# isl-org/adaptive-surface-reconstruction

Measured on AMD Instinct MI355X. Metric: input points/sec to signed implicit values, higher is better.
Workload: dtype f32 via bf16x3 (24-bit operands, f32 accumulate)

## Files before the change

adaptive-surface-reconstruction_amd/csrc/asr_common.h:

```cpp
#pragma once
#include <hip/hip_runtime.h>

#include <cstdint>
#include <cstdio>
#include <map>
#include <string>
#include <tuple>
#include <vector>

#include "../../include/asr_hip.h"
#include "asr_pending.h"

typedef uint64_t u64;
typedef int64_t i64;
typedef uint32_t u32;

struct Arena {
    struct Slab {
        char* base;
        size_t size, used;
    };
    std::vector<Slab> slabs;
    size_t min_slab = size_t(256) << 20;
    size_t cap = 0;
    uint64_t generation = 0;

    void* alloc(size_t bytes) {
        bytes = (bytes + 255) & ~size_t(255);
        if (bytes == 0) bytes = 256;
        for (auto& s : slabs)
            if (s.size - s.used >= bytes) {
                void* p = s.base + s.used;
                s.used += bytes;
                return p;
            }
        size_t sz = bytes > min_slab ? bytes : min_slab;
        if (cap && reserved() + sz > cap) return nullptr;
        void* p = nullptr;
        if (hipMalloc(&p, sz) != hipSuccess) return nullptr;
        slabs.push_back({(char*)p, sz, bytes});
        return p;
    }
    void reset() {
        for (auto& s : slabs) s.used = 0;
        ++generation;
    }
    size_t reserved() const {
        size_t t = 0;
        for (auto& s : slabs) t += s.size;
        return t;
    }
    void release() {
        for (auto& s : slabs) (void)hipFree(s.base);
        slabs.clear();
    }
};

struct ArenaMark {
    std::vector<size_t> used;
};
static inline void arena_mark(const Arena& a, ArenaMark& m) {
    m.used.clear();
    for (auto& s : a.slabs) m.used.push_back(s.used);
}
static inline void arena_rewind(Arena& a, const ArenaMark& m) {
    for (size_t i = 0; i < a.slabs.size(); ++i) a.slabs[i].used = i < m.used.size() ? m.used[i] : 0;
    ++a.generation;
}

struct GridDev {
    i64 v = 0, p = 0;
    u64* keys = nullptr;
    float* centers = nullptr;
    float* sizes = nullptr;
    int32_t* nidx = nullptr;
    uint8_t* nkidx = nullptr;
    i64* nrs = nullptr;
    int32_t* up_idx = nullptr;
    uint8_t* up_kidx = nullptr;
    i64* up_rs = nullptr;
    int32_t* down_idx = nullptr;
    uint8_t* down_kidx = nullptr;
    i64* down_rs = nullptr;
    int32_t* perm_nb = nullptr;
    int32_t* perm_up = nullptr;
    int32_t* perm_down = nullptr;
};

struct AsrOptions {
    i64 sconv_min_blocks = 2816;
    i64 sconv16_min_blocks = 1024;
    i64 sconv_wide_min = 2048;
    i64 row_segment = 524288;
    i64 search_hash_level = -1;
    i64 knn_deep = 1;
    i64 knn_cells = 1;
    i64 plan_arena = 0;
    i64 sconv_plan = 1;
    i64 row_ranked = 1;
    i64 row_lpt = 1;
    i64 overlap = 1;
    i64 cconv_valu = 0;
    i64 build_search = 1;
    i64 shard_geometry = -1;
    i64 shard_timing = 0;
    i64 search_priority = 2;
    i64 search_half = 1;
    i64 early_cells = 1;
    i64 early_sort = 1;
    i64 arena_cap_mb = 0;
    i64 inject_failure = 0;
    i64 sconv_split_min_rows = 2048;
    i64 sconv_split_rows = 32768;
};

struct asr_conv_plan_view {
    const uint4* hdr;
    const int32_t* pool;
    i64 groups;
    unsigned pool_bytes;
};
struct asr_conv_plan {
    uint4* hdr = nullptr;
    int32_t* pool = nullptr;
// ... 403 lines not shown
```

adaptive-surface-reconstruction_amd/csrc/asr_geom.hip:

```cpp
#include <cstdlib>
#include <cstring>
#include <algorithm>
#include <rocprim/rocprim.hpp>

#include "asr_common.h"
#include "asr_prim.h"

namespace {
using namespace asr_prim;

constexpr int BLK = 256;

struct HashTab {
    u64* keys;
    int32_t* vals;
    u64 mask;
};

struct TabProbe {
    u64 bucket, step, low, bmask;
    __device__ inline u64 slot() const { return ((bucket & bmask) << 6) | low; }
    __device__ inline void next() { bucket += step; }
};
__device__ inline TabProbe tab_probe(const HashTab& t, u64 key) {
    const u64 h = asr_hash64(key >> 6);
    return TabProbe{h, (h >> 32) | 1, key & 63, t.mask >> 6};
}

__device__ inline u64 ld_agent(const u64* p) {
    return __hip_atomic_load(p, __ATOMIC_RELAXED, __HIP_MEMORY_SCOPE_AGENT);
}

__device__ inline int tab_insert(const HashTab& t, u64 key, u64* slot_out = nullptr) {
    TabProbe pr = tab_probe(t, key);
    for (u64 probe = 0; probe <= pr.bmask; ++probe, pr.next()) {
        const u64 slot = pr.slot();
        u64 cur = ld_agent(&t.keys[slot]);
        if (cur == 0) {
            cur = atomicCAS((unsigned long long*)&t.keys[slot], 0ull, (unsigned long long)key);
            if (cur == 0) {
                if (slot_out) *slot_out = slot;
                return 1;
            }
        }
        if (cur == key) {
            if (slot_out) *slot_out = slot;
            return 0;
        }
    }
    return -1;
}
__device__ inline int tab_insert_shared(const HashTab& t, u64 key) {
    TabProbe pr = tab_probe(t, key);
    for (u64 probe = 0; probe <= pr.bmask; ++probe, pr.next()) {
        const u64 slot = pr.slot();
        u64 cur = t.keys[slot];
        if (cur == 0) cur = ld_agent(&t.keys[slot]);
        if (cur == 0) {
            cur = atomicCAS((unsigned long long*)&t.keys[slot], 0ull, (unsigned long long)key);
            if (cur == 0) return 1;
        }
        if (cur == key) return 0;
    }
    return -1;
}
__device__ inline bool tab_contains(const HashTab& t, u64 key) {
    TabProbe pr = tab_probe(t, key);
    for (u64 probe = 0; probe <= pr.bmask; ++probe, pr.next()) {
        const u64 slot = pr.slot();
        const u64 cur = t.keys[slot];
        if (cur == key) return true;
        if (cur == 0) return false;
    }
    return false;
}
__device__ inline int tab_find(const HashTab& t, u64 key) {
    TabProbe pr = tab_probe(t, key);
    for (u64 probe = 0; probe <= pr.bmask; ++probe, pr.next()) {
        const u64 slot = pr.slot();
        const u64 cur = t.keys[slot];
        if (cur == key) return t.vals[slot];
        if (cur == 0) return -1;
    }
    return -1;
}
__device__ inline i64 tab_find_slot(const HashTab& t, u64 key) {
    TabProbe pr = tab_probe(t, key);
    for (u64 probe = 0; probe <= pr.bmask; ++probe, pr.next()) {
        const u64 slot = pr.slot();
        const u64 cur = t.keys[slot];
        if (cur == key) return (i64)slot;
        if (cur == 0) return -1;
    }
    return -1;
// ... 105 lines not shown
            key = point_key(f, pts, radii, i, radius_scale, max_depth);
    }
    const u64 left = __shfl_up(key, 1, 64);
    if ((threadIdx.x & 63) != 0 && left == key) return;
    if (key == 0) return;
    insert_with_ancestors(t, key, cnt, list, list_cap);
}

__global__ void k_grow_init(asr_octree_frame f, const float* pts, const float* radii, i64 n, float radius_scale,
                            int max_depth, HashTab t, int* cnt, u64* list, int list_cap) {
    i64 i = blockIdx.x * (i64)blockDim.x + threadIdx.x;
    if (i >= n) return;
    if (!(isfinite(pts[3 * i]) && isfinite(pts[3 * i + 1]) && isfinite(pts[3 * i + 2]) && isfinite(radii[i]))) {
        cnt[F_NONFINITE] = 1;
        return;
    }
    const u64 key = point_key(f, pts, radii, i, radius_scale, max_depth);
    if (key == 0) return;
    const int r = tab_insert(t, key);
    if (r < 0) cnt[F_OVERFLOW] = 1;
    if (r == 1) {
        const int pos = atomicAdd(&cnt[F_ENTRIES], 1);
        if (pos < list_cap)
            list[pos] = key;
        else
            cnt[F_OVERFLOW] = 1;
    }
}
__device__ inline bool tab_has_child(const HashTab& t, u64 key) {
    if (__clzll((long long)key) <= 1) return false;
    for (int k = 0; k < 8; ++k)
        if (tab_contains(t, (key << 3) + k)) return true;
    return false;
}
__global__ void k_grow_candidates(HashTab t, const u64* list, int lo, int count, u64* cand) {
    const int e = blockIdx.x * blockDim.x + threadIdx.x;
    if (e >= count * 7) return;
    const u64 cur = list[lo + e / 7];
    u64 out = 0;
    if (cur != 1) {
        const int cfg = 7 - (int)(cur & 7);
        int j = e % 7;
        if (j >= cfg) ++j;
        int x, y, z, lev;
        asr_key_coord(cur >> 3, x, y, z, lev);
        const u64 key = asr_coord_key(x + (j & 1) - (cfg & 1), y + ((j >> 1) & 1) - ((cfg >> 1) & 1),
                                      z + ((j >> 2) & 1) - ((cfg >> 2) & 1), lev);
        if (key != 0 && !tab_contains(t, key) && !tab_has_child(t, key)) out = key;
    }
    cand[e] = out;
}
__global__ void k_grow_insert(HashTab t, u64* list, int lo, int count, const u64* cand, int* cnt, int list_cap) {
    const int e = blockIdx.x * blockDim.x + threadIdx.x;
    if (e >= count * 14) return;
    const u64 cur = list[lo + e / 14];
    if (cur == 1) return;
    const int j = e % 14;
    u64 key;
    if (j < 7) {
        key = cand[(e / 14) * 7 + j];
        if (key == 0) return;
    } else {
        const u64 first = cur & ~u64(7);
        int sj = j - 7;
        if (first + sj >= cur) ++sj;
        key = first + sj;
    }
    const int r = tab_insert(t, key);
    if (r < 0) cnt[F_OVERFLOW] = 1;
    if (r == 1) {
        const int pos = atomicAdd(&cnt[F_ENTRIES], 1);
        if (pos < list_cap)
            list[pos] = key;
        else
            cnt[F_OVERFLOW] = 1;
    }
}
__global__ void k_octree_insert_keys(const u64* keys, i64 n, HashTab t, int* cnt, u64* list, int list_cap) {
    i64 i = blockIdx.x * (i64)blockDim.x + threadIdx.x;
    if (i >= n) return;
    insert_with_ancestors(t, keys[i], cnt, list, list_cap);
}

__global__ void k_balance_classify(HashTab t, const u64* list, int lo, int ngroups, uint8_t* flag) {
    int i = blockIdx.x * blockDim.x + threadIdx.x;
    if (i >= ngroups) return;
    u64 k = list[lo + 8 * i];
    bool has_child = (__clzll((long long)k) > 1) && tab_contains(t, k << 3);
    flag[i] = has_child ? 0 : 1;
}
__global__ void k_balance_insert(HashTab t, u64* list, int lo, int ngroups, const uint8_t* flag,
                                 int* cnt, int list_cap) {
    int i = blockIdx.x * blockDim.x + threadIdx.x;
    if (i >= ngroups * 6) return;
    if (!flag[i / 6]) return;
    u64 k = list[lo + 8 * (i / 6)];
    int j = i % 6;
    const int ox = (j == 0) ? -1 : (j == 3) ? 1 : 0;
    const int oy = (j == 1) ? -1 : (j == 4) ? 1 : 0;
    const int oz = (j == 2) ? -1 : (j == 5) ? 1 : 0;
    int x, y, z, lev;
    asr_key_coord(k >> 3, x, y, z, lev);
    u64 key = asr_coord_key(x + ox, y + oy, z + oz, lev);
    if (key == 0) return;
    insert_with_ancestors(t, key, cnt, list, list_cap);
}
__global__ void k_leaf_flags(HashTab t, const u64* nodes, i64 n, uint8_t* flags) {
    i64 i = blockIdx.x * (i64)blockDim.x + threadIdx.x;
    if (i >= n) return;
    const u64 k = nodes[i];
    flags[i] = (k != 0 && !((__clzll((long long)k) > 1) && tab_contains(t, k << 3))) ? 1 : 0;
}

__global__ void k_leaf_tail(const u64* leaves, const i64* num, i64* out3) {
    const i64 n = *num;
    out3[0] = n;
    out3[1] = n > 0 ? (i64)leaves[0] : 0;
    out3[2] = n > 0 ? (i64)leaves[n - 1] : 0;
}

__global__ void k_map_build(const u64* keys, i64 v, HashTab t, int* cnt) {
    i64 i = blockIdx.x * (i64)blockDim.x + threadIdx.x;
    if (i >= v) return;
    u64 slot;
    int r = tab_insert(t, keys[i], &slot);
    if (r < 0)
        cnt[F_OVERFLOW] = 1;
    else
        t.vals[slot] = (int32_t)i;
}

__constant__ int8_t c_child_off[24][3] = {
        {-1, 0, 0}, {-1, 1, 0}, {-1, 0, 1}, {-1, 1, 1}, {2, 0, 0},  {2, 1, 0},  {2, 0, 1},  {2, 1, 1},
        {0, -1, 0}, {1, -1, 0}, {0, -1, 1}, {1, -1, 1}, {0, 2, 0},  {1, 2, 0},  {0, 2, 1},  {1, 2, 1},
        {0, 0, -1}, {1, 0, -1}, {0, 1, -1}, {1, 1, -1}, {0, 0, 2},  {1, 0, 2},  {0, 1, 2},  {1, 1, 2}};
__constant__ int8_t c_nb_off[6][3] = {{-1, 0, 0}, {1, 0, 0}, {0, -1, 0},
                                      {0, 1, 0},  {0, 0, -1}, {0, 0, 1}};
__constant__ int8_t c_parent_koff[6][8] = {
        {-1, 0, -1, 1, -1, 2, -1, 3}, {0, -1, 1, -1, 2, -1, 3, -1}, {-1, -1, 0, 1, -1, -1, 2, 3},
        {0, 1, -1, -1, 2, 3, -1, -1}, {-1, -1, -1, -1, 0, 1, 2, 3}, {0, 1, 2, 3, -1, -1, -1, -1}};

__device__ inline int neighbor_candidate(const HashTab& t, u64 key, int x, int y, int z, int lev,
                                         int c, int& slot) {
    if (c < 6) {
        u64 nk = asr_coord_key(x + c_nb_off[c][0], y + c_nb_off[c][1], z + c_nb_off[c][2], lev);
        slot = 1 + c;
        return nk ? tab_find(t, nk) : -1;
    } else if (c < 30) {
        if (lev >= ASR_MAX_LEVEL) return -1;
        int j = c - 6;
        u64 nk = asr_coord_key(2 * x + c_child_off[j][0], 2 * y + c_child_off[j][1],
                               2 * z + c_child_off[j][2], lev + 1);
        slot = 7 + j;
        return nk ? tab_find(t, nk) : -1;
    } else {
        if (lev <= 0) return -1;
        int j = c - 30;
        u64 nk = asr_coord_key(x + c_nb_off[j][0], y + c_nb_off[j][1], z + c_nb_off[j][2], lev);
        if (!nk) return -1;
        int koff = c_parent_koff[j][nk & 7];
        if (koff < 0) return -1;
        slot = 31 + 4 * j + koff;
        return tab_find(t, nk >> 3);
    }
}

__global__ void k_check_rows(const int32_t* rows, i64 nrows, i64 v, int* cnt, int32_t* mark) {
    const i64 r = blockIdx.x * (i64)blockDim.x + threadIdx.x;
    if (r >= nrows) return;
    const i64 q = rows[r];
    if (q < 0 || q >= v || (r > 0 && rows[r - 1] >= q)) cnt[F_BAD_KEY] = 1;
    else if (mark) mark[q] = 1;
}
__global__ void k_check_keys(const u64* keys, i64 n, int* cnt) {
    const i64 i = blockIdx.x * (i64)blockDim.x + threadIdx.x;
    if (i >= n) return;
    const u64 k = keys[i];
    if (k == 0 || (63 - __clzll((long long)k)) % 3 != 0) cnt[F_BAD_KEY] = 1;
}

constexpr int NB_STAGE = 16;
constexpr int NB_MAX_JOBS = 8;
struct NbBatch {
    int n;
    i64 base[NB_MAX_JOBS + 1];
    i64 v[NB_MAX_JOBS];
    const u64* keys[NB_MAX_JOBS];
    HashTab tab[NB_MAX_JOBS];
    i64* rs[NB_MAX_JOBS];
// ... 1896 lines not shown
    t.keys = arena_alloc<u64>(arena, cap);
    t.vals = with_vals ? arena_alloc<int32_t>(arena, cap) : nullptr;
    t.mask = cap - 1;
    if (!t.keys || (with_vals && !t.vals)) ASR_FAIL(ctx, ASR_HIP_EHIP, "arena allocation failed");
    ASR_HIP_CHECK(ctx, hipMemsetAsync(t.keys, 0, cap * sizeof(u64), ctx->stream));
    return ASR_HIP_OK;
}

}

int asr_geom_point_keys(asr_hip_context* ctx, const asr_octree_frame* frame, const float* pts,
                        const float* radii, i64 n, float radius_scale, int max_depth, u64* keys) {
    if (n <= 0) return ASR_HIP_OK;
    k_point_keys<<<grid_for(n, BLK), BLK, 0, ctx->stream>>>(*frame, pts, radii, n, radius_scale,
                                                            max_depth, keys);
    ASR_CHECK_LAUNCH(ctx);
    return ASR_HIP_OK;
}

static int grow_keys(asr_hip_context* ctx, Arena& arena, const asr_octree_frame* frame, const float* pts, const float* radii,
                     i64 n, float radius_scale, int max_depth, int grow_steps, u64** keys_out, i64* count_out) {
    HostFlags host;
    u64 cap = next_pow2((u64)std::max<i64>(i64(1) << 16, 8 * n));
    for (int attempt = 0; attempt < 6; ++attempt, cap <<= 2) {
        if (attempt) ++ctx->table_regrows;
        HashTab t;
        ASR_TRY(make_table(ctx, arena, cap, false, t));
        const int lcap = (int)std::min<u64>(cap / 2, u64(1) << 30);
        u64* list = arena_alloc<u64>(arena, (size_t)lcap + 8);
        if (!list) ASR_FAIL(ctx, ASR_HIP_EHIP, "arena allocation failed");
        ASR_TRY(fresh_flags(ctx));
        k_grow_init<<<grid_for(n, BLK), BLK, 0, ctx->stream>>>(*frame, pts, radii, n, radius_scale, max_depth, t,
                                                             ctx->d_flags, list, lcap);
        ASR_CHECK_LAUNCH(ctx);
        ASR_TRY(read_flags(ctx, host));
        if (host[F_BAD_KEY]) ASR_FAIL(ctx, ASR_HIP_EINVAL, "octree: extra_keys holds a value that is no location code (0 or a leading "
                                                   "bit that is not at 3 * level)");
        if (host[F_NONFINITE]) ASR_FAIL(ctx, ASR_HIP_EINVAL, "octree: points / radii contain non-finite values");
        bool overflow = host[F_OVERFLOW] != 0;
        int lo = 0, hi = host[F_ENTRIES];
        for (int it = 0; it < grow_steps && !overflow && hi > lo; ++it) {
            const int count = hi - lo;
            if ((i64)count * 14 >= (i64(1) << 31) || (u64)(hi + (i64)count * 14) > (u64)lcap) {
                overflow = true;
                break;
            }
            u64* cand = arena_alloc<u64>(arena, (size_t)count * 7);
            if (!cand) ASR_FAIL(ctx, ASR_HIP_EHIP, "arena allocation failed");
            k_grow_candidates<<<grid_for((i64)count * 7, BLK), BLK, 0, ctx->stream>>>(t, list, lo, count, cand);
            ASR_CHECK_LAUNCH(ctx);
            k_grow_insert<<<grid_for((i64)count * 14, BLK), BLK, 0, ctx->stream>>>(t, list, lo, count, cand, ctx->d_flags,
                                                                                  lcap);
            ASR_CHECK_LAUNCH(ctx);
            ASR_TRY(read_flags(ctx, host));
            overflow = host[F_OVERFLOW] != 0;
            lo = hi;
            hi = host[F_ENTRIES];
        }
        if (overflow) continue;
        *keys_out = list;
        *count_out = host[F_ENTRIES];
        return ASR_HIP_OK;
    }
    ASR_FAIL(ctx, ASR_HIP_ELOGIC, "octree grow: hash table overflow");
}

int asr_geom_octree_build(asr_hip_context* ctx, const asr_octree_frame* frame, const float* pts,
                          const float* radii, i64 n, float radius_scale, int max_depth, int grow_steps,
                          const u64* extra_keys, i64 num_extra, bool balance) {
    ASR_TRY(ensure_flags(ctx));
    if (max_depth > ASR_MAX_LEVEL) max_depth = ASR_MAX_LEVEL;
    if (max_depth < 0) ASR_FAIL(ctx, ASR_HIP_EINVAL, "max_depth must be >= 0");
    if (grow_steps < 0) ASR_FAIL(ctx, ASR_HIP_EINVAL, "grow_steps must be >= 0");
    u64* grown = nullptr;
    i64 num_grown = 0;
    Arena grow_arena;
    grow_arena.min_slab = size_t(16) << 20;
    struct ArenaGuard {
        Arena& a;
        ~ArenaGuard() { a.release(); }
    } grow_guard{grow_arena};
    if (grow_steps > 0 && n > 0)
        ASR_TRY(grow_keys(ctx, grow_arena, frame, pts, radii, n, radius_scale, max_depth, grow_steps, &grown, &num_grown));
    u64 cap = next_pow2((u64)std::max<i64>(i64(1) << 16, 2 * std::max(std::max(n, 4 * num_grown), num_extra)));
    HostFlags host;
    for (int attempt = 0; attempt < 7; ++attempt, cap <<= 2) {
        if (attempt) ++ctx->table_regrows;
        ctx->scratch.reset();
        HashTab t;
        ASR_TRY(make_table(ctx, ctx->scratch, cap, false, t));
        int lcap = (int)std::min<u64>(cap / 2, u64(1) << 30);
        u64* list = arena_alloc<u64>(ctx->scratch, (size_t)lcap + 8);
        uint8_t* flag = arena_alloc<uint8_t>(ctx->scratch, (size_t)lcap / 8 + 8);
        if (!list || !flag) ASR_FAIL(ctx, ASR_HIP_EHIP, "arena allocation failed");
        ASR_TRY(fresh_flags(ctx));
        if (grown) {
            if (num_grown > 0)
                k_octree_insert_keys<<<grid_for(num_grown, BLK), BLK, 0, ctx->stream>>>(grown, num_grown, t, ctx->d_flags,
                                                                                       list, lcap);
            ASR_CHECK_LAUNCH(ctx);
        } else if (n > 0) {
            k_octree_insert_points<<<grid_for(n, BLK), BLK, 0, ctx->stream>>>(*frame, pts, radii, n, radius_scale, max_depth,
                                                                              t, ctx->d_flags, list, lcap);
            ASR_CHECK_LAUNCH(ctx);
        }
        if (num_extra > 0) {
            k_check_keys<<<grid_for(num_extra, BLK), BLK, 0, ctx->stream>>>(extra_keys, num_extra, ctx->d_flags);
            ASR_CHECK_LAUNCH(ctx);
            k_octree_insert_keys<<<grid_for(num_extra, BLK), BLK, 0, ctx->stream>>>(extra_keys, num_extra, t, ctx->d_flags,
                                                                                   list, lcap);
            ASR_CHECK_LAUNCH(ctx);
        }
        k_list_key_bits<<<256, BLK, 0, ctx->stream>>>(list, lcap, ctx->d_flags);
        ASR_CHECK_LAUNCH(ctx);
        ASR_TRY(read_flags(ctx, host));
        if (host[F_NONFINITE]) ASR_FAIL(ctx, ASR_HIP_EINVAL, "octree: points / radii contain non-finite values");
        bool overflow = host[F_OVERFLOW] != 0 || (u64)host[F_ENTRIES] * 2 > cap;
        int lo = 0, hi = host[F_ENTRIES];
        while (balance && !overflow && hi > lo) {
            int ngroups = (hi - lo) / 8;
            k_balance_classify<<<grid_for(ngroups, BLK), BLK, 0, ctx->stream>>>(t, list, lo, ngroups, flag);
            ASR_CHECK_LAUNCH(ctx);
            k_balance_insert<<<grid_for((i64)ngroups * 6, BLK), BLK, 0, ctx->stream>>>(
                    t, list, lo, ngroups, flag, ctx->d_flags, lcap);
            ASR_CHECK_LAUNCH(ctx);
            ASR_TRY(read_flags(ctx, host));
            overflow = host[F_OVERFLOW] != 0 || (u64)host[F_ENTRIES] * 2 > cap;
            lo = hi;
            hi = host[F_ENTRIES];
        }
        if (overflow) continue;
        i64 num_nodes = (i64)host[F_ENTRIES] + (host[F_ROOT] ? 1 : 0);
        ctx->leaf_lmin = ctx->leaf_lmax = -1;
        if (num_nodes == 0) {
            ctx->num_nodes = ctx->num_leaves = 0;
            ctx->nodes = ctx->leaves = nullptr;
            return ASR_HIP_OK;
        }
        if (host[F_ROOT]) {
            const u64 one = 1;
            ASR_HIP_CHECK(ctx, hipMemcpyAsync(list + host[F_ENTRIES], &one, sizeof(u64), hipMemcpyHostToDevice,
                                              ctx->stream));
        }
        ctx->nodes = arena_alloc<u64>(ctx->persist, num_nodes);
        u64* leaves_tmp = arena_alloc<u64>(ctx->scratch, num_nodes);
        uint8_t* lflag = arena_alloc<uint8_t>(ctx->scratch, num_nodes);
        i64* d_num = arena_alloc<i64>(ctx->scratch, 1);
        if (!ctx->nodes || !leaves_tmp || !lflag || !d_num) ASR_FAIL(ctx, ASR_HIP_EHIP, "arena allocation failed");
        ASR_TRY(sort_keys(ctx, ctx->scratch, list, ctx->nodes, num_nodes, host[F_KEY_BITS] > 0 && host[F_KEY_BITS] <= 64 ? host[F_KEY_BITS] : 64));
        k_leaf_flags<<<grid_for(num_nodes, BLK), BLK, 0, ctx->stream>>>(t, ctx->nodes, num_nodes, lflag);
        ASR_CHECK_LAUNCH(ctx);
        {
            size_t tb = 0;
            ASR_HIP_CHECK(ctx, rocprim::select(nullptr, tb, ctx->nodes, lflag, leaves_tmp, d_num, (size_t)num_nodes,
                                               ctx->stream));
            void* tmp = ctx->scratch.alloc(tb ? tb : 256);
            if (!tmp) ASR_FAIL(ctx, ASR_HIP_EHIP, "arena allocation failed");
            ASR_HIP_CHECK(ctx, rocprim::select(tmp, tb, ctx->nodes, lflag, leaves_tmp, d_num, (size_t)num_nodes,
                                               ctx->stream));
        }
        i64* d_tail = arena_alloc<i64>(ctx->scratch, 3);
        if (!d_tail) ASR_FAIL(ctx, ASR_HIP_EHIP, "arena allocation failed");
        k_leaf_tail<<<1, 1, 0, ctx->stream>>>(leaves_tmp, d_num, d_tail);
        ASR_CHECK_LAUNCH(ctx);
        i64 tail[3] = {0, 0, 0};
        ASR_HIP_CHECK(ctx, hipMemcpyAsync(tail, d_tail, sizeof(tail), hipMemcpyDeviceToHost, ctx->stream));
        ASR_HIP_CHECK(ctx, hipStreamSynchronize(ctx->stream));
        const i64 num_leaves = tail[0];
        auto level_of = [](u64 k) { return k ? (63 - __builtin_clzll(k)) / 3 : 0; };
        ctx->leaf_lmin = level_of((u64)tail[1]);
        ctx->leaf_lmax = level_of((u64)tail[2]);
        ctx->leaves = arena_alloc<u64>(ctx->persist, num_leaves);
        if (!ctx->leaves) ASR_FAIL(ctx, ASR_HIP_EHIP, "arena allocation failed");
        ASR_HIP_CHECK(ctx, hipMemcpyAsync(ctx->leaves, leaves_tmp, 8 * num_leaves, hipMemcpyDeviceToDevice, ctx->stream));
        ctx->num_nodes = num_nodes;
        ctx->num_leaves = num_leaves;
        return ASR_HIP_OK;
    }
    ASR_FAIL(ctx, ASR_HIP_ELOGIC, "octree hash table overflow after 6 growth attempts");
}

template <class Pass>
static int nb_key_maps(asr_hip_context* ctx, NbBatch& b, Pass&& pass, int grow0 = 0, int* grow_out = nullptr) {
    ASR_TRY(ensure_flags(ctx));
    for (int grow = grow0;; grow += 2) {
        u64 caps[NB_MAX_JOBS], cap_sum = 0;
        for (int j = 0; j < b.n; ++j) {
            caps[j] = next_pow2((u64)std::max<i64>(1024, 2 * b.v[j])) << grow;
            cap_sum += caps[j];
        }
        u64* tkeys = arena_alloc<u64>(ctx->scratch, cap_sum);
        int32_t* tvals = arena_alloc<int32_t>(ctx->scratch, cap_sum);
        if (!tkeys || !tvals) ASR_FAIL(ctx, ASR_HIP_EHIP, "arena allocation failed");
        u64 off = 0;
        for (int j = 0; j < b.n; ++j) {
            b.tab[j] = HashTab{tkeys + off, tvals + off, caps[j] - 1};
            off += caps[j];
        }
        ASR_HIP_CHECK(ctx, hipMemsetAsync(tkeys, 0, cap_sum * sizeof(u64), ctx->stream));
        ASR_TRY(fresh_flags(ctx));
        k_map_build_batch<<<grid_for(b.base[b.n], BLK), BLK, 0, ctx->stream>>>(b, ctx->d_flags);
        ASR_CHECK_LAUNCH(ctx);
        ASR_TRY(pass());
        HostFlags host;
        ASR_TRY(read_flags(ctx, host));
        if (!host[F_OVERFLOW]) {
            if (grow_out) *grow_out = grow;
            return ASR_HIP_OK;
        }
        if (grow >= 6) ASR_FAIL(ctx, ASR_HIP_ELOGIC, "voxel key map overflow");
        ++ctx->table_regrows;
    }
}

static NbBatch nb_one_grid(const u64* keys, i64 v) {
    NbBatch b;
    b.n = 1;
    b.base[0] = 0;
    b.base[1] = v + 1;
    b.v[0] = v;
    b.keys[0] = keys;
    b.rs[0] = nullptr;
    b.idx[0] = nullptr;
    b.kidx[0] = nullptr;
    b.owner[0] = nullptr;
    b.me[0] = 1;
    return b;
}

static int check_row_list(asr_hip_context* ctx, const int32_t* rows, i64 nrows, i64 v, int32_t* mark = nullptr) {
    ASR_TRY(ensure_flags(ctx));
    ASR_HIP_CHECK(ctx, hipMemsetAsync(ctx->d_flags + F_BAD_KEY, 0, sizeof(int), ctx->stream));
    k_check_rows<<<grid_for(nrows, BLK), BLK, 0, ctx->stream>>>(rows, nrows, v, ctx->d_flags, mark);
    ASR_CHECK_LAUNCH(ctx);
    HostFlags host;
    ASR_TRY(read_flags(ctx, host));
    if (host[F_BAD_KEY]) ASR_FAIL(ctx, ASR_HIP_EINVAL, "neighbour rows: the row list must be strictly ascending indices in [0, %lld)", (long long)v);
    return ASR_HIP_OK;
}

int asr_geom_grid_neighbors_count(asr_hip_context* ctx, const u64* keys, i64 v, const int32_t* rows, i64 nrows, i64* rs,
                                  i64* num_pairs) {
    *num_pairs = 0;
    if (v <= 0) {
        ASR_HIP_CHECK(ctx, hipMemsetAsync(rs, 0, sizeof(i64), ctx->stream));
        return ASR_HIP_OK;
    }
    ctx->nb_grow_keys = nullptr;
    NbBatch b = nb_one_grid(keys, v);
    if (rows) {
        int32_t* mark = arena_alloc<int32_t>(ctx->scratch, v);
        if (!mark) ASR_FAIL(ctx, ASR_HIP_EHIP, "arena allocation failed");
        ASR_HIP_CHECK(ctx, hipMemsetAsync(mark, 0, v * sizeof(int32_t), ctx->stream));
        ASR_TRY(check_row_list(ctx, rows, nrows, v, mark));
        b.owner[0] = mark;
    }
    i64* counts = arena_alloc<i64>(ctx->scratch, v + 1);
    if (!counts) ASR_FAIL(ctx, ASR_HIP_EHIP, "arena allocation failed");
    ASR_TRY(nb_key_maps(ctx, b, [&]() -> int {
        k_neighbors_count_batch<<<grid_for(v + 1, BLK), BLK, 0, ctx->stream>>>(b, counts, nullptr, nullptr, nullptr);
        ASR_CHECK_LAUNCH(ctx);
        return scan_counts(ctx, ctx->scratch, counts, rs, v + 1);
// ... 1327 lines not shown
```

adaptive-surface-reconstruction_amd/csrc/asr_prim.h:

```cpp
#pragma once
#include <rocprim/rocprim.hpp>

#include "asr_common.h"

namespace asr_prim {

constexpr int FLAG_BLOCK = 64, FLAG_BLOCKS = 512;
enum Flag : int {
    F_ENTRIES = 0,
    F_OVERFLOW = 1,
    F_MASKS = 2,
    F_BAD_KEY = 3,
    F_BAD_INDEX = 4,
    F_BAD_LEVEL = 5,
    F_LEVEL_MIN = 6,
    F_LEVEL_MAX = 7,
    F_POINT_LEVEL = 8,
    F_ROOT = 9,
    F_HEAVY = 10,
    F_NONFINITE = 11,
    F_KNN_CELLS = 12,
    F_KNN_FALLBACK = 13,
    F_MAX_CELL_POP = 14,
    F_MARGIN_PAIRS = 15,
    F_DUAL_FAN = 16,
    F_DUAL_SORT = 17,
    F_OUTSIDE = 18,
    F_BAD_VERTEX = 19,
    F_KEY_BITS = 20,
    F_DUAL_KEY = 21,
    F_CELLS = 22,
    F_MERGE_DROPPED = 23,
    F_MERGE_SPLIT = 24,
    F_MERGE_CLUSTERS = 25,
    F_MERGE_LARGEST = 26,
    F_MERGE_LONG = 27,
    F_ORIENT_SKIPPED = 28,
    F_ORIENT_FLIPPED = 29,
    F_ORIENT_TREES = 30,
    F_ORIENT_HOOKED = 31,
    F_COUNT
};
constexpr int FLAG_READ = 32;
constexpr int FLAG_LEVEL_CELLS = 32;
static_assert(F_COUNT <= FLAG_READ, "read_flags must cover every slot");
static_assert(FLAG_READ <= FLAG_LEVEL_CELLS && FLAG_LEVEL_CELLS + ASR_MAX_LEVEL + 1 <= FLAG_BLOCK,
              "the per-level cell counts lie behind the slots, inside the block");
static_assert(F_LEVEL_MAX == F_LEVEL_MIN + 1, "query_level_range sets both with one copy");
static_assert(F_KNN_FALLBACK == F_KNN_CELLS + 1, "asr_geom_knn clears both with one memset");
struct HostFlags {
    int v[FLAG_READ];
    int operator[](Flag f) const { return v[f]; }
};
static inline int ensure_flags(asr_hip_context* ctx) {
    if (!ctx->d_flags_base) {
        ASR_HIP_CHECK(ctx, hipMalloc((void**)&ctx->d_flags_base, (size_t)FLAG_BLOCK * FLAG_BLOCKS * sizeof(int)));
        ASR_HIP_CHECK(ctx, hipMemsetAsync(ctx->d_flags_base, 0, (size_t)FLAG_BLOCK * FLAG_BLOCKS * sizeof(int), ctx->stream));
        ctx->d_flags = ctx->d_flags_base;
        ctx->flags_next = 1;
    }
    return ASR_HIP_OK;
}
static inline int fresh_flags(asr_hip_context* ctx) {
    ASR_TRY(ensure_flags(ctx));
    if (ctx->flags_next >= FLAG_BLOCKS) {
        ASR_HIP_CHECK(ctx, hipMemsetAsync(ctx->d_flags_base, 0, (size_t)FLAG_BLOCK * FLAG_BLOCKS * sizeof(int), ctx->stream));
        ctx->flags_next = 0;
    }
    ctx->d_flags = ctx->d_flags_base + (size_t)FLAG_BLOCK * ctx->flags_next++;
    return ASR_HIP_OK;
}
static inline int count_begin(asr_hip_context* ctx) {
    pending_begin(ctx->pending);
    ctx->scratch.reset();
    return fresh_flags(ctx);
}
static inline int count_done(asr_hip_context* ctx, PendingOp op) {
    pending_commit(ctx->pending, op, ctx->scratch.generation);
    return ASR_HIP_OK;
}
static inline bool fill_begin(asr_hip_context* ctx, PendingOp op) {
    return pending_claim(ctx->pending, op, ctx->scratch.generation);
}
#define SCRATCH_ALLOC(var, T, count)                        \
    T* var = arena_alloc<T>(ctx->scratch, (size_t)(count)); \
    if (!var) ASR_FAIL(ctx, ASR_HIP_EHIP, "arena allocation failed")
static inline int read_flags(asr_hip_context* ctx, HostFlags& host) {
    ASR_HIP_CHECK(ctx, hipMemcpyAsync(host.v, ctx->d_flags, FLAG_READ * sizeof(int), hipMemcpyDeviceToHost,
                                      ctx->stream));
    ASR_HIP_CHECK(ctx, hipStreamSynchronize(ctx->stream));
    return ASR_HIP_OK;
}

static inline int sort_keys(asr_hip_context* ctx, Arena& arena, const u64* in, u64* out, i64 n, int end_bit = 64) {
    if (n <= 0) return ASR_HIP_OK;
    size_t tb = 0;
    ASR_HIP_CHECK(ctx, rocprim::radix_sort_keys(nullptr, tb, in, out, (size_t)n, 0, end_bit,
                                                ctx->stream));
    void* tmp = arena.alloc(tb ? tb : 256);
    if (!tmp) ASR_FAIL(ctx, ASR_HIP_EHIP, "arena allocation failed");
    ASR_HIP_CHECK(ctx, rocprim::radix_sort_keys(tmp, tb, in, out, (size_t)n, 0, end_bit,
                                                ctx->stream));
    return ASR_HIP_OK;
}
template <class K, class V>
static inline int sort_pairs(asr_hip_context* ctx, Arena& arena, const K* kin, K* kout, const V* vin, V* vout,
               i64 n, int end_bit, int begin_bit = 0) {
    if (n <= 0) return ASR_HIP_OK;
    size_t tb = 0;
    ASR_HIP_CHECK(ctx, rocprim::radix_sort_pairs(nullptr, tb, kin, kout, vin, vout, (size_t)n, begin_bit,
                                                 end_bit, ctx->stream));
    void* tmp = arena.alloc(tb ? tb : 256);
    if (!tmp) ASR_FAIL(ctx, ASR_HIP_EHIP, "arena allocation failed");
    ASR_HIP_CHECK(ctx, rocprim::radix_sort_pairs(tmp, tb, kin, kout, vin, vout, (size_t)n, begin_bit,
                                                 end_bit, ctx->stream));
    return ASR_HIP_OK;
}
static inline int scan_counts(asr_hip_context* ctx, Arena& arena, const i64* in, i64* out, i64 n_plus_1) {
    size_t tb = 0;
    ASR_HIP_CHECK(ctx, rocprim::exclusive_scan(nullptr, tb, in, out, i64(0), (size_t)n_plus_1,
                                               rocprim::plus<i64>(), ctx->stream));
    void* tmp = arena.alloc(tb ? tb : 256);
    if (!tmp) ASR_FAIL(ctx, ASR_HIP_EHIP, "arena allocation failed");
    ASR_HIP_CHECK(ctx, rocprim::exclusive_scan(tmp, tb, in, out, i64(0), (size_t)n_plus_1,
                                               rocprim::plus<i64>(), ctx->stream));
    return ASR_HIP_OK;
}
// ... 26 lines not shown
```

Before: 271.5 million.

## Batch octree balance rounds on device to cut host syncs per round

Balance iterations now keep the frontier bounds in device flag slots, advanced by a one-thread kernel, so several classify/insert rounds can be queued before one host readback, replacing a sync after every round. The classify and insert kernels become grid-stride loops with capped grids that read their work bounds from device memory. The root key is written by a tiny kernel instead of a host-to-device copy, and leaves are selected straight into persistent memory whose unused tail is returned, dropping a device-to-device copy. Extra rounds past convergence launch empty kernels, and the capped grids may under-parallelise large frontiers.

```diff
diff --git a/adaptive-surface-reconstruction_amd/csrc/asr_common.h b/adaptive-surface-reconstruction_amd/csrc/asr_common.h
--- a/adaptive-surface-reconstruction_amd/csrc/asr_common.h
+++ b/adaptive-surface-reconstruction_amd/csrc/asr_common.h
@@ -40,6 +40,18 @@
         if (hipMalloc(&p, sz) != hipSuccess) return nullptr;
         slabs.push_back({(char*)p, sz, bytes});
         return p;
+    }
+    bool shrink_last(const void* p, size_t old_bytes, size_t new_bytes) {
+        auto rounded = [](size_t b) { return b ? (b + 255) & ~size_t(255) : size_t(256); };
+        old_bytes = rounded(old_bytes);
+        new_bytes = rounded(new_bytes);
+        if (new_bytes > old_bytes) return false;
+        for (auto& s : slabs)
+            if ((const char*)p >= s.base && s.used >= old_bytes && (const char*)p == s.base + (s.used - old_bytes)) {
+                s.used -= old_bytes - new_bytes;
+                return true;
+            }
+        return false;
     }
     void reset() {
         for (auto& s : slabs) s.used = 0;
diff --git a/adaptive-surface-reconstruction_amd/csrc/asr_frontier.h b/adaptive-surface-reconstruction_amd/csrc/asr_frontier.h
--- /dev/null
+++ b/adaptive-surface-reconstruction_amd/csrc/asr_frontier.h
@@ -0,0 +1,35 @@
+#pragma once
+
+namespace asr_frontier {
+
+constexpr int BATCH = 4;
+
+struct State {
+    int entries = 0, lo = 0, hi = 0;
+    bool overflow = false;
+};
+
+template <class Enqueue, class Read>
+static inline int run(int batch, bool iterate, Enqueue&& enqueue, Read&& read, State& s, int* reads = nullptr) {
+    if (batch < 1) batch = 1;
+    for (;;) {
+        if (iterate)
+            for (int b = 0; b < batch; ++b)
+                if (int rc = enqueue()) return rc;
+        if (int rc = read(s)) return rc;
+        if (reads) ++*reads;
+        if (s.overflow || !iterate || s.entries <= s.hi) return 0;
+    }
+}
+
+template <class Attempt>
+static inline int run_growing(int attempts, Attempt&& attempt, State& s) {
+    for (int a = 0; a < attempts; ++a) {
+        s = State();
+        if (int rc = attempt(a, s)) return rc;
+        if (!s.overflow) return 0;
+    }
+    return 0;
+}
+
+}
diff --git a/adaptive-surface-reconstruction_amd/csrc/asr_geom.hip b/adaptive-surface-reconstruction_amd/csrc/asr_geom.hip
--- a/adaptive-surface-reconstruction_amd/csrc/asr_geom.hip
+++ b/adaptive-surface-reconstruction_amd/csrc/asr_geom.hip
@@ -4,12 +4,14 @@
 #include <rocprim/rocprim.hpp>
 
 #include "asr_common.h"
+#include "asr_frontier.h"
 #include "asr_prim.h"
 
 namespace {
 using namespace asr_prim;
 
 constexpr int BLK = 256;
+constexpr unsigned BALANCE_MAX_BLOCKS = 4096;
 
 struct HashTab {
     u64* keys;
@@ -281,29 +283,35 @@
     insert_with_ancestors(t, keys[i], cnt, list, list_cap);
 }
 
-__global__ void k_balance_classify(HashTab t, const u64* list, int lo, int ngroups, uint8_t* flag) {
-    int i = blockIdx.x * blockDim.x + threadIdx.x;
-    if (i >= ngroups) return;
-    u64 k = list[lo + 8 * i];
-    bool has_child = (__clzll((long long)k) > 1) && tab_contains(t, k << 3);
-    flag[i] = has_child ? 0 : 1;
-}
-__global__ void k_balance_insert(HashTab t, u64* list, int lo, int ngroups, const uint8_t* flag,
-                                 int* cnt, int list_cap) {
-    int i = blockIdx.x * blockDim.x + threadIdx.x;
-    if (i >= ngroups * 6) return;
-    if (!flag[i / 6]) return;
-    u64 k = list[lo + 8 * (i / 6)];
-    int j = i % 6;
-    const int ox = (j == 0) ? -1 : (j == 3) ? 1 : 0;
-    const int oy = (j == 1) ? -1 : (j == 4) ? 1 : 0;
-    const int oz = (j == 2) ? -1 : (j == 5) ? 1 : 0;
-    int x, y, z, lev;
-    asr_key_coord(k >> 3, x, y, z, lev);
-    u64 key = asr_coord_key(x + ox, y + oy, z + oz, lev);
-    if (key == 0) return;
-    insert_with_ancestors(t, key, cnt, list, list_cap);
-}
+__global__ void k_balance_advance(int* cnt, int list_cap) {
+    cnt[F_FRONT_LO] = cnt[F_FRONT_HI];
+    cnt[F_FRONT_HI] = min(cnt[F_ENTRIES], list_cap);
+}
+__global__ void k_balance_classify(HashTab t, const u64* list, const int* cnt, uint8_t* flag) {
+    const int lo = cnt[F_FRONT_LO], ngroups = (cnt[F_FRONT_HI] - lo) / 8;
+    for (int i = blockIdx.x * blockDim.x + threadIdx.x; i < ngroups; i += gridDim.x * blockDim.x) {
+        u64 k = list[lo + 8 * i];
+        bool has_child = (__clzll((long long)k) > 1) && tab_contains(t, k << 3);
+        flag[i] = has_child ? 0 : 1;
+    }
+}
+__global__ void k_balance_insert(HashTab t, u64* list, const uint8_t* flag, int* cnt, int list_cap) {
+    const int lo = cnt[F_FRONT_LO], nwork = (cnt[F_FRONT_HI] - lo) / 8 * 6;
+    for (int i = blockIdx.x * blockDim.x + threadIdx.x; i < nwork; i += gridDim.x * blockDim.x) {
+        if (!flag[i / 6]) continue;
+        u64 k = list[lo + 8 * (i / 6)];
+        int j = i % 6;
+        const int ox = (j == 0) ? -1 : (j == 3) ? 1 : 0;
+        const int oy = (j == 1) ? -1 : (j == 4) ? 1 : 0;
+        const int oz = (j == 2) ? -1 : (j == 5) ? 1 : 0;
+        int x, y, z, lev;
+        asr_key_coord(k >> 3, x, y, z, lev);
+        u64 key = asr_coord_key(x + ox, y + oy, z + oz, lev);
+        if (key == 0) continue;
+        insert_with_ancestors(t, key, cnt, list, list_cap);
+    }
+}
+__global__ void k_list_root(u64* list, int entries) { list[entries] = 1; }
 __global__ void k_leaf_flags(HashTab t, const u64* nodes, i64 n, uint8_t* flags) {
     i64 i = blockIdx.x * (i64)blockDim.x + threadIdx.x;
     if (i >= n) return;
@@ -2366,15 +2374,17 @@
     } grow_guard{grow_arena};
     if (grow_steps > 0 && n > 0)
         ASR_TRY(grow_keys(ctx, grow_arena, frame, pts, radii, n, radius_scale, max_depth, grow_steps, &grown, &num_grown));
-    u64 cap = next_pow2((u64)std::max<i64>(i64(1) << 16, 2 * std::max(std::max(n, 4 * num_grown), num_extra)));
+    const u64 cap0 = next_pow2((u64)std::max<i64>(i64(1) << 16, 2 * std::max(std::max(n, 4 * num_grown), num_extra)));
     HostFlags host;
-    for (int attempt = 0; attempt < 7; ++attempt, cap <<= 2) {
+    HashTab t;
+    u64* list = nullptr;
+    auto closure = [&](int attempt, asr_frontier::State& front) -> int {
+        const u64 cap = cap0 << (2 * attempt);
         if (attempt) ++ctx->table_regrows;
         ctx->scratch.reset();
-        HashTab t;
         ASR_TRY(make_table(ctx, ctx->scratch, cap, false, t));
-        int lcap = (int)std::min<u64>(cap / 2, u64(1) << 30);
-        u64* list = arena_alloc<u64>(ctx->scratch, (size_t)lcap + 8);
+        const int lcap = (int)std::min<u64>(cap / 2, u64(1) << 30);
+        list = arena_alloc<u64>(ctx->scratch, (size_t)lcap + 8);
         uint8_t* flag = arena_alloc<uint8_t>(ctx->scratch, (size_t)lcap / 8 + 8);
         if (!list || !flag) ASR_FAIL(ctx, ASR_HIP_EHIP, "arena allocation failed");
         ASR_TRY(fresh_flags(ctx));
@@ -2397,71 +2407,75 @@
         }
         k_list_key_bits<<<256, BLK, 0, ctx->stream>>>(list, lcap, ctx->d_flags);
         ASR_CHECK_LAUNCH(ctx);
-        ASR_TRY(read_flags(ctx, host));
+        const unsigned classify_grid = std::min<unsigned>(grid_for(lcap / 8, BLK), BALANCE_MAX_BLOCKS);
+        const unsigned insert_grid = std::min<unsigned>(grid_for((i64)(lcap / 8) * 6, BLK), BALANCE_MAX_BLOCKS);
+        auto balance_round = [&]() -> int {
+            k_balance_advance<<<1, 1, 0, ctx->stream>>>(ctx->d_flags, lcap);
+            ASR_CHECK_LAUNCH(ctx);
+            k_balance_classify<<<classify_grid, BLK, 0, ctx->stream>>>(t, list, ctx->d_flags, flag);
+            ASR_CHECK_LAUNCH(ctx);
+            k_balance_insert<<<insert_grid, BLK, 0, ctx->stream>>>(t, list, flag, ctx->d_flags, lcap);
+            ASR_CHECK_LAUNCH(ctx);
+            return ASR_HIP_OK;
+        };
+        auto read_frontier = [&](asr_frontier::State& s) -> int {
+            ASR_TRY(read_flags(ctx, host));
+            s.entries = host[F_ENTRIES];
+            s.lo = host[F_FRONT_LO];
+            s.hi = host[F_FRONT_HI];
+            s.overflow = host[F_OVERFLOW] != 0 || (u64)host[F_ENTRIES] * 2 > cap;
+            return ASR_HIP_OK;
+        };
+        ASR_TRY(asr_frontier::run(asr_frontier::BATCH, balance, balance_round, read_frontier, front));
         if (host[F_NONFINITE]) ASR_FAIL(ctx, ASR_HIP_EINVAL, "octree: points / radii contain non-finite values");
-        bool overflow = host[F_OVERFLOW] != 0 || (u64)host[F_ENTRIES] * 2 > cap;
-        int lo = 0, hi = host[F_ENTRIES];
-        while (balance && !overflow && hi > lo) {
-            int ngroups = (hi - lo) / 8;
-            k_balance_classify<<<grid_for(ngroups, BLK), BLK, 0, ctx->stream>>>(t, list, lo, ngroups, flag);
-            ASR_CHECK_LAUNCH(ctx);
-            k_balance_insert<<<grid_for((i64)ngroups * 6, BLK), BLK, 0, ctx->stream>>>(
-                    t, list, lo, ngroups, flag, ctx->d_flags, lcap);
-            ASR_CHECK_LAUNCH(ctx);
-            ASR_TRY(read_flags(ctx, host));
-            overflow = host[F_OVERFLOW] != 0 || (u64)host[F_ENTRIES] * 2 > cap;
-            lo = hi;
-            hi = host[F_ENTRIES];
-        }
-        if (overflow) continue;
-        i64 num_nodes = (i64)host[F_ENTRIES] + (host[F_ROOT] ? 1 : 0);
-        ctx->leaf_lmin = ctx->leaf_lmax = -1;
-        if (num_nodes == 0) {
-            ctx->num_nodes = ctx->num_leaves = 0;
-            ctx->nodes = ctx->leaves = nullptr;
-            return ASR_HIP_OK;
-        }
-        if (host[F_ROOT]) {
-            const u64 one = 1;
-            ASR_HIP_CHECK(ctx, hipMemcpyAsync(list + host[F_ENTRIES], &one, sizeof(u64), hipMemcpyHostToDevice,
-                                              ctx->stream));
-        }
-        ctx->nodes = arena_alloc<u64>(ctx->persist, num_nodes);
-        u64* leaves_tmp = arena_alloc<u64>(ctx->scratch, num_nodes);
-        uint8_t* lflag = arena_alloc<uint8_t>(ctx->scratch, num_nodes);
-        i64* d_num = arena_alloc<i64>(ctx->scratch, 1);
-        if (!ctx->nodes || !leaves_tmp || !lflag || !d_num) ASR_FAIL(ctx, ASR_HIP_EHIP, "arena allocation failed");
-        ASR_TRY(sort_keys(ctx, ctx->scratch, list, ctx->nodes, num_nodes, host[F_KEY_BITS] > 0 && host[F_KEY_BITS] <= 64 ? host[F_KEY_BITS] : 64));
-        k_leaf_flags<<<grid_for(num_nodes, BLK), BLK, 0, ctx->stream>>>(t, ctx->nodes, num_nodes, lflag);
+        return ASR_HIP_OK;
+    };
+    asr_frontier::State front;
+    ASR_TRY(asr_frontier::run_growing(7, closure, front));
+    if (front.overflow) ASR_FAIL(ctx, ASR_HIP_ELOGIC, "octree hash table overflow after 6 growth attempts");
+    i64 num_nodes = (i64)host[F_ENTRIES] + (host[F_ROOT] ? 1 : 0);
+    ctx->leaf_lmin = ctx->leaf_lmax = -1;
+    if (num_nodes == 0) {
+        ctx->num_nodes = ctx->num_leaves = 0;
+        ctx->nodes = ctx->leaves = nullptr;
+        return ASR_HIP_OK;
+    }
+    if (host[F_ROOT]) {
+        k_list_root<<<1, 1, 0, ctx->stream>>>(list, host[F_ENTRIES]);
         ASR_CHECK_LAUNCH(ctx);
-        {
-            size_t tb = 0;
-            ASR_HIP_CHECK(ctx, rocprim::select(nullptr, tb, ctx->nodes, lflag, leaves_tmp, d_num, (size_t)num_nodes,
-                                               ctx->stream));
-            void* tmp = ctx->scratch.alloc(tb ? tb : 256);
-            if (!tmp) ASR_FAIL(ctx, ASR_HIP_EHIP, "arena allocation failed");
-            ASR_HIP_CHECK(ctx, rocprim::select(tmp, tb, ctx->nodes, lflag, leaves_tmp, d_num, (size_t)num_nodes,
-                                               ctx->stream));
-        }
-        i64* d_tail = arena_alloc<i64>(ctx->scratch, 3);
-        if (!d_tail) ASR_FAIL(ctx, ASR_HIP_EHIP, "arena allocation failed");
-        k_leaf_tail<<<1, 1, 0, ctx->stream>>>(leaves_tmp, d_num, d_tail);
-        ASR_CHECK_LAUNCH(ctx);
-        i64 tail[3] = {0, 0, 0};
-        ASR_HIP_CHECK(ctx, hipMemcpyAsync(tail, d_tail, sizeof(tail), hipMemcpyDeviceToHost, ctx->stream));
-        ASR_HIP_CHECK(ctx, hipStreamSynchronize(ctx->stream));
-        const i64 num_leaves = tail[0];
-        auto level_of = [](u64 k) { return k ? (63 - __builtin_clzll(k)) / 3 : 0; };
-        ctx->leaf_lmin = level_of((u64)tail[1]);
-        ctx->leaf_lmax = level_of((u64)tail[2]);
-        ctx->leaves = arena_alloc<u64>(ctx->persist, num_leaves);
-        if (!ctx->leaves) ASR_FAIL(ctx, ASR_HIP_EHIP, "arena allocation failed");
-        ASR_HIP_CHECK(ctx, hipMemcpyAsync(ctx->leaves, leaves_tmp, 8 * num_leaves, hipMemcpyDeviceToDevice, ctx->stream));
-        ctx->num_nodes = num_nodes;
-        ctx->num_leaves = num_leaves;
-        return ASR_HIP_OK;
-    }
-    ASR_FAIL(ctx, ASR_HIP_ELOGIC, "octree hash table overflow after 6 growth attempts");
+    }
+    ctx->nodes = arena_alloc<u64>(ctx->persist, num_nodes);
+    ctx->leaves = arena_alloc<u64>(ctx->persist, num_nodes);
+    uint8_t* lflag = arena_alloc<uint8_t>(ctx->scratch, num_nodes);
+    i64* d_num = arena_alloc<i64>(ctx->scratch, 1);
+    if (!ctx->nodes || !ctx->leaves || !lflag || !d_num) ASR_FAIL(ctx, ASR_HIP_EHIP, "arena allocation failed");
+    ASR_TRY(sort_keys(ctx, ctx->scratch, list, ctx->nodes, num_nodes, host[F_KEY_BITS] > 0 && host[F_KEY_BITS] <= 64 ? host[F_KEY_BITS] : 64));
+    k_leaf_flags<<<grid_for(num_nodes, BLK), BLK, 0, ctx->stream>>>(t, ctx->nodes, num_nodes, lflag);
+    ASR_CHECK_LAUNCH(ctx);
+    {
+        size_t tb = 0;
+        ASR_HIP_CHECK(ctx, rocprim::select(nullptr, tb, ctx->nodes, lflag, ctx->leaves, d_num, (size_t)num_nodes, ctx->stream));
+        void* tmp = ctx->scratch.alloc(tb ? tb : 256);
+        if (!tmp) ASR_FAIL(ctx, ASR_HIP_EHIP, "arena allocation failed");
+        ASR_HIP_CHECK(ctx, rocprim::select(tmp, tb, ctx->nodes, lflag, ctx->leaves, d_num, (size_t)num_nodes, ctx->stream));
+    }
+    i64* d_tail = arena_alloc<i64>(ctx->scratch, 3);
+    if (!d_tail) ASR_FAIL(ctx, ASR_HIP_EHIP, "arena allocation failed");
+    k_leaf_tail<<<1, 1, 0, ctx->stream>>>(ctx->leaves, d_num, d_tail);
+    ASR_CHECK_LAUNCH(ctx);
+    i64 tail[3] = {0, 0, 0};
+    ASR_HIP_CHECK(ctx, hipMemcpyAsync(tail, d_tail, sizeof(tail), hipMemcpyDeviceToHost, ctx->stream));
+    ASR_HIP_CHECK(ctx, hipStreamSynchronize(ctx->stream));
+    const i64 num_leaves = tail[0];
+    auto level_of = [](u64 k) { return k ? (63 - __builtin_clzll(k)) / 3 : 0; };
+    ctx->leaf_lmin = level_of((u64)tail[1]);
+    ctx->leaf_lmax = level_of((u64)tail[2]);
+    if (num_leaves < 0 || num_leaves > num_nodes ||
+        !ctx->persist.shrink_last(ctx->leaves, 8 * (size_t)num_nodes, 8 * (size_t)num_leaves))
+        ASR_FAIL(ctx, ASR_HIP_ELOGIC, "octree: cannot give back the unused tail of the leaves");
+    ctx->num_nodes = num_nodes;
+    ctx->num_leaves = num_leaves;
+    return ASR_HIP_OK;
 }
 
 template <class Pass>
diff --git a/adaptive-surface-reconstruction_amd/csrc/asr_prim.h b/adaptive-surface-reconstruction_amd/csrc/asr_prim.h
--- a/adaptive-surface-reconstruction_amd/csrc/asr_prim.h
+++ b/adaptive-surface-reconstruction_amd/csrc/asr_prim.h
@@ -39,10 +39,12 @@
     F_ORIENT_FLIPPED = 29,
     F_ORIENT_TREES = 30,
     F_ORIENT_HOOKED = 31,
+    F_FRONT_LO = 32,
+    F_FRONT_HI = 33,
     F_COUNT
 };
-constexpr int FLAG_READ = 32;
-constexpr int FLAG_LEVEL_CELLS = 32;
+constexpr int FLAG_READ = 40;
+constexpr int FLAG_LEVEL_CELLS = 40;
 static_assert(F_COUNT <= FLAG_READ, "read_flags must cover every slot");
 static_assert(FLAG_READ <= FLAG_LEVEL_CELLS && FLAG_LEVEL_CELLS + ASR_MAX_LEVEL + 1 <= FLAG_BLOCK,
               "the per-level cell counts lie behind the slots, inside the block");
```

Result: no change. 272.2 million, median of 2 (+0.3%).
